# rvp-group/mad-icp

Hardware: NVIDIA H100
Metric: scans/sec (130k-pt scan vs 16-keyframe model) (higher is better)
Workload: dtype f64

## Files before the change

### include/madicp_b200.h

```cpp
#ifndef MADICP_B200_H
#define MADICP_B200_H

#include <stddef.h>
#include <stdint.h>

#ifdef __cplusplus
extern "C" {
#endif

#define MADICP_OK 0
#define MADICP_ERR_INVALID (-1)
#define MADICP_ERR_CUDA (-2)
#define MADICP_ERR_STATE (-3)
#define MADICP_ERR_NOMEM (-4)
#define MADICP_ERR_COMM (-5)

#define MADICP_MAX_ITERS 64

typedef struct madtree_rec {
  double mean[3];
  double dir[3];
  double bbox0;
  int32_t link;
  int32_t num_points;
// ... 56 lines not shown
int madicp_get_moving(madicp_ctx_t* ctx, double* means_out, int cap_leaves);
int madicp_put_keyframe_tree(madicp_ctx_t* ctx, int slot, const madtree_gpu_t* t, const double X[12]);

int madicp_ingest(madicp_ctx_t* ctx, const void* xyz, int64_t n, int is_f32, int deskew, const double T_prev[12],
                  const double T_now[12], double sensor_hz, int num_threads, double* points_out);

int madicp_search(madicp_ctx_t* ctx, const double X[12], int32_t* out_ordinals);

int madicp_linearize(madicp_ctx_t* ctx, const double X[12], double H[36], double b[6], uint8_t* matched);

int madicp_solve_update(madicp_ctx_t* ctx, const double H[36], const double b[6], double X_inout[12]);

int madicp_register(madicp_ctx_t* ctx, int iters, double X_inout[12], double H_last[36], double b_last[6],
                    uint8_t* matched_last, int* n_matched);
int madicp_register_async(madicp_ctx_t* ctx, int iters, const double X0[12]);
int madicp_register_fetch(madicp_ctx_t* ctx, double X[12], double H_last[36], double b_last[6], uint8_t* matched_last,
                          int* n_matched);
int madicp_register_fetch_weight(madicp_ctx_t* ctx, double X[12], double H_last[36], double b_last[6],
                                 uint8_t* matched_last, int* n_matched, double* weight);
int madicp_register_partial_async(madicp_ctx_t* ctx, int iters, const double X0[12]);
int madicp_register_trace(madicp_ctx_t* ctx, double* X_trace, int max_rounds);

int madicp_register_walked(madicp_ctx_t* ctx, int32_t* walked, int max_rounds);

int madicp_deskew(double* points_xyz, int64_t n, const double T_prev[12], const double T_now[12], double sensor_hz,
                  int num_threads);

int madicp_search_cloud(madicp_ctx_t* ctx, int slot, const double* queries_xyz, int64_t n, int32_t* ordinals,
                        double* points, double* normals, double* dists);

int64_t madicp_kernel_launches(const madicp_ctx_t* ctx);
int64_t madicp_model_nodes(const madicp_ctx_t* ctx);

#define MADICP_IPC_HANDLE_BYTES 64
int madicp_comm_export(madicp_ctx_t* ctx, void* handle_out );
int madicp_comm_connect(madicp_ctx_t* ctx, int rank, int world, const void* all_handles );
int madicp_comm_world(const madicp_ctx_t* ctx);

int madicp_calibrate(madicp_ctx_t* ctx, const double X0[12]);


#ifdef __cplusplus
}
#endif
#endif
```

### include/madicp_b200_debug.h

```cpp
#ifndef MADICP_B200_DEBUG_H
#define MADICP_B200_DEBUG_H

#include "madicp_b200.h"

#ifdef __cplusplus
extern "C" {
#endif

int madicp_debug_timing(madicp_ctx_t* ctx, int enable, int64_t* out, int max_rounds);
int madicp_debug_cta_cycles(madicp_ctx_t* ctx, int64_t* out, int cap);
int madicp_debug_cta_stamps(madicp_ctx_t* ctx, int plane, int64_t* out, int cap);
int madicp_set_gn_grid(madicp_ctx_t* ctx, int threads_per_cta, int ctas_per_sm);


int madicp_debug_set_memo(madicp_ctx_t* ctx, int enable);

int64_t madicp_debug_sort_check(int64_t n, uint32_t seed, int64_t distinct, int num_threads);

#ifdef __cplusplus
}
#endif
#endif
```

### mad_icp_b200/_capi.py

```python
import ctypes as C
import os

import numpy as np

_HERE = os.path.dirname(os.path.abspath(__file__))
LIB_PATH = os.path.join(_HERE, "lib", "libmadicp_b200.so")
_lib = None

dp = C.POINTER(C.c_double)
ip = C.POINTER(C.c_int32)
bp = C.POINTER(C.c_uint8)
vp = C.c_void_p

SYMBOLS = {
    "madicp_last_error": (C.c_char_p, []),
    "madicp_abi_version": (C.c_int, []),
    "madtree_build": (C.c_int, [dp, C.c_int64, C.c_double, C.c_double, C.c_int, C.POINTER(vp)]),
    "madtree_free": (None, [vp]),
    "madtree_num_nodes": (C.c_int, [vp]),
    "madtree_num_leaves": (C.c_int, [vp]),
    "madtree_apply_transform": (C.c_int, [vp, dp]),
    "madtree_leaves": (C.c_int, [vp, dp, dp, dp, ip]),
    "madtree_records": (vp, [vp]),
    "madtree_num_levels": (C.c_int, [vp]),
# ... 22 lines not shown
    "madtree_gpu_num_leaves": (C.c_int, [vp]),
    "madtree_gpu_num_levels": (C.c_int, [vp]),
    "madtree_gpu_download": (C.c_int, [vp, vp, ip]),
    "madtree_gpu_export": (C.c_int, [vp, dp, dp, dp, ip]),
    "madicp_set_moving_tree": (C.c_int, [vp, vp]),
    "madicp_get_moving": (C.c_int, [vp, dp, C.c_int]),
    "madicp_ingest": (C.c_int, [vp, vp, C.c_int64, C.c_int, C.c_int, dp, dp, C.c_double, C.c_int, dp]),
    "madicp_register_fetch_weight": (C.c_int, [vp, dp, dp, dp, bp, C.POINTER(C.c_int), dp]),
    "madicp_register_partial_async": (C.c_int, [vp, C.c_int, dp]),
    "madicp_calibrate": (C.c_int, [vp, dp]),
    "madicp_drop_keyframe": (C.c_int, [vp, C.c_int]),
    "madicp_num_keyframes": (C.c_int, [vp]),
    "madicp_active_slots": (C.c_int, [vp, ip, C.c_int]),
    "madicp_keyframe_leaves": (C.c_int, [vp, C.c_int]),
    "madicp_set_moving": (C.c_int, [vp, vp, C.c_int]),
    "madicp_search": (C.c_int, [vp, dp, ip]),
    "madicp_linearize": (C.c_int, [vp, dp, dp, dp, bp]),
    "madicp_solve_update": (C.c_int, [vp, dp, dp, dp]),
    "madicp_register": (C.c_int, [vp, C.c_int, dp, dp, dp, bp, C.POINTER(C.c_int)]),
    "madicp_register_async": (C.c_int, [vp, C.c_int, dp]),
    "madicp_register_fetch": (C.c_int, [vp, dp, dp, dp, bp, C.POINTER(C.c_int)]),
    "madicp_register_trace": (C.c_int, [vp, dp, C.c_int]),
    "madicp_register_walked": (C.c_int, [vp, ip, C.c_int]),
    "madicp_search_cloud": (C.c_int, [vp, C.c_int, dp, C.c_int64, ip, dp, dp, dp]),
    "madicp_deskew": (C.c_int, [dp, C.c_int64, dp, dp, C.c_double, C.c_int]),
    "madicp_debug_sort_check": (C.c_int64, [C.c_int64, C.c_uint32, C.c_int64, C.c_int]),
    "madicp_kernel_launches": (C.c_int64, [vp]),
    "madicp_model_nodes": (C.c_int64, [vp]),
    "madicp_comm_export": (C.c_int, [vp, vp]),
    "madicp_comm_connect": (C.c_int, [vp, C.c_int, C.c_int, vp]),
    "madicp_comm_world": (C.c_int, [vp]),
    "madicp_debug_timing": (C.c_int, [vp, C.c_int, C.POINTER(C.c_int64), C.c_int]),
    "madicp_debug_cta_cycles": (C.c_int, [vp, C.POINTER(C.c_int64), C.c_int]),
    "madicp_set_gn_grid": (C.c_int, [vp, C.c_int, C.c_int]),
    "madicp_debug_set_memo": (C.c_int, [vp, C.c_int]),
    "madicp_debug_cta_stamps": (C.c_int, [vp, C.c_int, C.POINTER(C.c_int64), C.c_int]),
}

REC_DTYPE = np.dtype([("mean", "<f8", 3), ("dir", "<f8", 3), ("bbox0", "<f8"), ("link", "<i4"), ("num_points", "<i4")])
assert REC_DTYPE.itemsize == 64


class MadIcpError(RuntimeError):
    pass


# ... 43 lines not shown
```

### mad_icp_b200/csrc/capi.cu

```cuda
#include <cooperative_groups.h>
#include <cuda_runtime.h>

#include <algorithm>
#include <cmath>
#include <cstdio>
#include <cstdlib>
#include <cstring>
#include <new>
#include <stdexcept>
#include <string>
#include <vector>

#include "../../include/madicp_b200_debug.h"
#include "ctx.hpp"
#include "device_kernels.cuh"

namespace madicp {

static thread_local std::string g_error;
void set_error(const std::string& msg) { g_error = msg; }

}

using namespace madicp;
// ... 218 lines not shown
  c->max_keyframes = max_keyframes;
  c->sm_count = prop.multiProcessorCount;
  c->slots.resize(max_keyframes);
  {
    int lo_pri = 0, hi_pri = 0;
    CK(cudaDeviceGetStreamPriorityRange(&lo_pri, &hi_pri));
    CK(cudaStreamCreateWithPriority(&c->own_stream, cudaStreamNonBlocking, hi_pri));
  }
  c->stream = c->own_stream;
  CK(cudaMalloc(&c->d_state, sizeof(GnState)));
  CK(cudaMemset(c->d_state, 0, sizeof(GnState)));
  CK(cudaMalloc(&c->d_X, sizeof(double) * 64));
  CK(cudaMalloc(&c->d_comm, sizeof(CommBlock)));
  CK(cudaMemset(c->d_comm, 0, sizeof(CommBlock)));
  CK(cudaEventCreateWithFlags(&c->tree_free_ev, cudaEventDisableTiming));
  CK(cudaMalloc(&c->d_pool_lvl, size_t(max_keyframes) * (kMaxLevels + 1) * sizeof(int)));
  CK(cudaMalloc(&c->d_xform, size_t(madicp_ctx::kXformRing) * 12 * sizeof(double)));
  CK(cudaMallocHost(&c->h_xform, size_t(madicp_ctx::kXformRing) * 12 * sizeof(double)));
  CK(cudaMallocHost(&c->h_lvl, size_t(madicp_ctx::kXformRing) * (kMaxLevels + 1) * sizeof(int)));
  for (int i = 0; i < madicp_ctx::kXformRing; ++i) CK(cudaEventCreateWithFlags(&c->xform_done[i], cudaEventDisableTiming));
  CK(cudaMallocHost(&c->h_pinned, sizeof(double) * 64));
  CK(cudaMallocHost(&c->h_state, sizeof(GnState)));
  CK(cudaMallocHost(&c->h_matched, kMatchedCap));
  if (const char* e = getenv("MADICP_NO_MEMO")) c->use_memo = (atoi(e) == 0);
  int threads = 1024, ctas = 1;
  if (const char* e = getenv("MADICP_GN_SHAPE"))
    if (sscanf(e, "%d,%d", &threads, &ctas) == 2) c->gn_auto = false;
  int rc = configure_gn(c, threads, ctas);
  if (rc) return rc;
  c->cap_partial = size_t(c->sm_count) * 8 * kAcc;
  CK(cudaMalloc(&c->d_partial, c->cap_partial * sizeof(double)));
  CK(cudaMalloc(&c->d_tiles, c->cap_partial * sizeof(LLCell)));
  CK(cudaMemset(c->d_tiles, 0, c->cap_partial * sizeof(LLCell)));
  c->peer_comm[0] = c->d_comm;
  *out = c;
  return MADICP_OK;
  MADICP_CATCH("madicp_create")
}

void madicp_destroy(madicp_ctx_t* c) {
  if (!c) return;
  cudaSetDevice(c->device);
  cudaStreamSynchronize(c->stream);
  for (int r = 0; r < c->world; ++r)
    if (c->world > 1 && r != c->rank && c->peer_comm[r]) cudaIpcCloseMemHandle(c->peer_comm[r]);
  madicp_gpu_build_release(c);
  for (madtree_gpu* t : c->tree_cache) delete t;
  for (void* slab : c->tree_slabs) cudaFree(slab);
  cudaFree(c->d_pool_recs);
  cudaFree(c->d_pool_child0);
  cudaFree(c->d_pool_rec_of);
  cudaFree(c->d_pool_lvl);
  cudaFree(c->d_quad);
  cudaFree(c->d_pool_ww);
  cudaFree(c->d_xform);
  cudaFree(c->d_dbg_cta);
  cudaFree(c->d_moving);
  cudaFree(c->d_mov4);
  cudaFree(c->d_step_matched);
  cudaFree(c->d_hit);
  cudaFree(c->d_ord);
  cudaFree(c->d_cloud_q);
  cudaFree(c->d_cloud_o);
  cudaFree(c->d_partial);
  cudaFree(c->d_tiles);
  cudaFree(c->d_memo_leaf);
  cudaFree(c->d_memo_margin);
  cudaFree(c->d_state);
  cudaFree(c->d_X);
  cudaFree(c->d_comm);
  cudaFree(c->d_dbg);
  cudaFreeHost(c->h_xform);
  cudaFreeHost(c->h_lvl);
  cudaFreeHost(c->h_pinned);
  cudaFreeHost(c->h_state);
  for (int i = 0; i < madicp_ctx::kXformRing; ++i)
    if (c->xform_done[i]) cudaEventDestroy(c->xform_done[i]);
  cudaFreeHost(c->h_matched);
  if (c->tree_free_ev) cudaEventDestroy(c->tree_free_ev);
  cudaStreamDestroy(c->own_stream);
  delete c;
}

int madicp_set_params(madicp_ctx_t* c, double min_ball, double rho_ker, double b_ratio) {
  if (!c || !(min_ball > 0) || rho_ker < 0) {
    set_error("madicp_set_params: bad arguments");
    return MADICP_ERR_INVALID;
  }
  const bool reweigh = (min_ball != c->P.min_ball);
  c->P.min_ball = min_ball;
// ... 503 lines not shown
  A.clear_from = clear_from;
  A.matched = c->d_comm->matched[mb];
  size_t map_bytes = 0;
  {
    const size_t per_cta = size_t(madicp_num_keyframes(c)) * (size_t(c->L) / size_t(c->gn_grid) + 8) * 4 + 128;
    auto bucket = [](size_t bytes) {
      const size_t kb[] = {8, 16, 32, 64, 100, 132, 164, 196, 228};
      for (size_t b : kb)
        if (bytes + 1024 <= b * 1024) return b;
      return size_t(1 << 20);
    };
    const size_t ctas = size_t(c->gn_grid / c->sm_count);
    if (per_cta <= kGnMapMaxBytes && c->L < (1 << 26) && bucket((c->gn_smem + per_cta) * ctas) == bucket(c->gn_smem * ctas))
      map_bytes = per_cta;
  }
  A.map_in_smem = map_bytes ? 1 : 0;
  {
    const size_t stride = ((size_t(c->max_keyframes) * (c->cap_moving / size_t(c->gn_grid) + 8)) + 31) & ~size_t(31);
    const size_t need = stride * size_t(c->gn_grid);
    if (need > c->cap_memo) {
      CK(cudaStreamSynchronize(c->stream));
      cudaFree(c->d_memo_leaf);
      cudaFree(c->d_memo_margin);
      c->d_memo_leaf = nullptr;
      c->d_memo_margin = nullptr;
      c->cap_memo = 0;
      const size_t cap = need + need / 4;
      CK(cudaMalloc(&c->d_memo_leaf, cap * sizeof(int)));
      CK(cudaMalloc(&c->d_memo_margin, cap * sizeof(float)));
      c->cap_memo = cap;
    }
    A.memo_leaf = c->d_memo_leaf;
    A.memo_margin = c->d_memo_margin;
    A.item_stride = int(stride);
    A.use_memo = c->use_memo ? 1 : 0;
    A.walk_buf = mb;
  }
  A.st = c->d_state;
  A.dbg = c->d_dbg;
  A.dbg_cta = c->d_dbg ? c->d_dbg_cta : nullptr;
  c->epoch += uint32_t(iters);
  A.pose_epoch = c->pose_epoch;
  c->pose_epoch += uint32_t(iters);
  memcpy(A.X0, X0, 12 * sizeof(double));
  A.tiles = c->d_tiles;
  A.zero_next = c->d_comm->matched[mb ^ 1];
  A.zero_bytes = int((std::min(kMatchedCap, c->cap_moving) + 15) & ~size_t(15));
  void* args[] = {&A};
  CK(cudaLaunchCooperativeKernel(c->gn_kernel, dim3(c->gn_grid), dim3(c->gn_threads), args, c->gn_smem + map_bytes, c->stream));
  c->launches++;
  c->last_iters = iters;
  c->call_seq++;
  return MADICP_OK;
}

int madicp_register_async(madicp_ctx_t* c, int iters, const double X0[12]) {
  return register_enqueue(c, iters, X0, iters - 1);
}
// ... 56 lines not shown
  return madicp_register_fetch(c, X, H, b, matched, n_matched);
}

int madicp_register_trace(madicp_ctx_t* c, double* X_trace, int max_rounds) {
  if (!c || !X_trace || c->last_iters < 1) return MADICP_ERR_INVALID;
  CK(cudaSetDevice(c->device));
  int rows = c->last_iters + 1;
  if (rows > max_rounds) rows = max_rounds;
  CK(cudaMemcpyAsync(c->h_state->X_trace, c->d_state->X_trace, size_t(rows) * 12 * sizeof(double),
                     cudaMemcpyDeviceToHost, c->stream));
  CK(cudaStreamSynchronize(c->stream));
  memcpy(X_trace, c->h_state->X_trace, size_t(rows) * 12 * sizeof(double));
  return rows;
}

int madicp_register_walked(madicp_ctx_t* c, int32_t* walked, int max_rounds) {
  if (!c || !walked || c->last_iters < 1) return MADICP_ERR_INVALID;
  CK(cudaSetDevice(c->device));
  int rows = std::min(c->last_iters, max_rounds);
  CK(cudaMemcpyAsync(c->h_state->walked[0], c->d_state->walked[(c->call_seq - 1u) & 1u], size_t(rows) * sizeof(int),
                     cudaMemcpyDeviceToHost, c->stream));
  CK(cudaStreamSynchronize(c->stream));
  memcpy(walked, c->h_state->walked[0], size_t(rows) * sizeof(int));
  return rows;
}

int madicp_search_cloud(madicp_ctx_t* c, int slot, const double* q, int64_t n, int32_t* ordinals, double* points,
                        double* normals, double* dists) {
  if (!c || !q || n < 1 || slot < 0 || slot >= c->max_keyframes || c->slots[slot].n_nodes == 0) {
    set_error("madicp_search_cloud: bad arguments or empty slot");
    return MADICP_ERR_INVALID;
  }
  CK(cudaSetDevice(c->device));
  if (size_t(n) > c->cap_cloud) {
    CK(cudaStreamSynchronize(c->stream));
    cudaFree(c->d_cloud_q);
    cudaFree(c->d_cloud_o);
    c->d_cloud_q = nullptr;
    c->d_cloud_o = nullptr;
    c->cap_cloud = 0;
    const size_t cap = size_t(n) + size_t(n) / 4 + 1024;
    CK(cudaMalloc(&c->d_cloud_q, cap * 10 * sizeof(double)));
    CK(cudaMalloc(&c->d_cloud_o, cap * sizeof(int)));
    c->cap_cloud = cap;
  }
  double* d_q = c->d_cloud_q;
// ... 124 lines not shown
  }
  return rows;
}

int madicp_debug_cta_cycles(madicp_ctx_t* c, int64_t* out, int cap) {
  if (!c || !out || !c->d_dbg_cta) return MADICP_ERR_INVALID;
  CK(cudaSetDevice(c->device));
  CK(cudaStreamSynchronize(c->stream));
  const int n = std::min(cap, c->last_iters * c->gn_grid);
  CK(cudaMemcpy(out, c->d_dbg_cta, size_t(n) * sizeof(long long), cudaMemcpyDeviceToHost));
  return c->gn_grid;
}

int madicp_debug_cta_stamps(madicp_ctx_t* c, int plane, int64_t* out, int cap) {
  if (!c || !out || !c->d_dbg_cta || plane < 0 || plane > 4) return MADICP_ERR_INVALID;
  CK(cudaSetDevice(c->device));
  CK(cudaStreamSynchronize(c->stream));
  const int n = std::min(cap, c->last_iters * c->gn_grid);
  CK(cudaMemcpy(out, c->d_dbg_cta + size_t(plane) * MADICP_MAX_ITERS * c->gn_grid, size_t(n) * sizeof(long long),
                cudaMemcpyDeviceToHost));
  return c->gn_grid;
}

int madicp_debug_set_memo(madicp_ctx_t* c, int enable) {
  if (!c) return MADICP_ERR_INVALID;
  c->use_memo = enable != 0;
  return MADICP_OK;
}

int madicp_set_gn_grid(madicp_ctx_t* c, int threads_per_cta, int ctas_per_sm) {
  if (!c || ctas_per_sm < 1) return MADICP_ERR_INVALID;
  CK(cudaSetDevice(c->device));
  if (threads_per_cta == 0) {
    c->gn_auto = true;
    return 0;
  }
  int rc = configure_gn(c, threads_per_cta, ctas_per_sm);
  if (rc) return rc;
  c->gn_auto = false;
  return c->gn_grid / c->sm_count;
}

}
```

### mad_icp_b200/csrc/ctx.hpp

```cpp
#pragma once
#include <cuda_runtime.h>

#include <atomic>
#include <mutex>
#include <new>
#include <stdexcept>
#include <string>
#include <vector>

#include "kernels.cuh"

namespace madicp {
void set_error(const std::string& msg);

constexpr int kMaxLevels = 4096;
struct Slot {
  int n_nodes = 0, n_leaves = 0, n_levels = 0;
};
constexpr size_t kMatchedCap = size_t(1) << 20;

struct CommBlock {
  Mailbox box;
  unsigned char matched[2][kMatchedCap];
};
// ... 40 lines not shown
  cudaEvent_t tree_free_ev = nullptr;
  std::mutex tree_mu;
  void* build_state = nullptr;
  long long* d_dbg_cta = nullptr;
  madicp::IcpParams P{0.2, 0.31622776601683794, 0.02};
  double* d_moving = nullptr;
  madicp::Moving4* d_mov4 = nullptr;
  bool mov4_stale = true;
  unsigned char* d_step_matched = nullptr;
  int L = 0;
  size_t cap_moving = 0;
  uint32_t call_seq = 0;
  int* d_hit = nullptr;
  int* d_ord = nullptr;
  size_t cap_items = 0;
  double* d_cloud_q = nullptr;
  int* d_cloud_o = nullptr;
  size_t cap_cloud = 0;
  double* d_partial = nullptr;
  madicp::LLCell* d_tiles = nullptr;
  size_t cap_partial = 0;
  int* d_memo_leaf = nullptr;
  float* d_memo_margin = nullptr;
  size_t cap_memo = 0;
  bool use_memo = true;
  madicp::GnState* d_state = nullptr;
  double* d_X = nullptr;
  madicp::CommBlock* d_comm = nullptr;
  double* h_pinned = nullptr;
  madicp::GnState* h_state = nullptr;
  unsigned char* h_matched = nullptr;
  int gn_grid = 0;
  bool gn_auto = true;
  int gn_threads = 1024;
  const void* gn_kernel = nullptr;
  size_t gn_smem = 0;
  static constexpr int kNumAutoShapes = 6;
  static constexpr int kAutoShapes[kNumAutoShapes] = {768, 1024, 896, 704, 640, 512};
  double pass_cost[kNumAutoShapes] = {5570.0, 8260.0, 7480.0, 5650.0, 5325.0, 4650.0};
  bool calibrated = false;
  int last_iters = 0;
  long long* d_dbg = nullptr;
  std::atomic<int64_t> launches{0};
  int rank = 0, world = 1;
  madicp::CommBlock* peer_comm[madicp::kMaxPeers] = {};
  uint32_t epoch = 0;
  uint32_t pose_epoch = 1;
};
// ... 25 lines not shown
```

### mad_icp_b200/csrc/device_kernels.cuh

```cuda
#pragma once
#include "kernels.cuh"

namespace madicp {


__device__ __forceinline__ int depth_of(const int* __restrict__ lvl, int n_levels, int i) {
  int lo = 0, hi = n_levels;
  while (hi - lo > 1) {
    const int mid = (lo + hi) >> 1;
    if (__ldg(lvl + mid) <= i) lo = mid; else hi = mid;
  }
  return lo;
}

__global__ void __launch_bounds__(kStepBlock)
k_slot_ingest(const madtree_rec_t* src, madtree_rec_t* dst, int n, const double* __restrict__ Xp,
              const int* __restrict__ lvl, int n_levels, int* __restrict__ flag) {
  const int i = blockIdx.x * kStepBlock + threadIdx.x;
  if (i >= n) return;
  Rec r = load_rec_plain(src + i);
  const int npts = src[i].num_points;
  int f = 0;
  if (r.link >= 0 && (depth_of(lvl, n_levels, i) & 1) == 0)
    f = (src[r.link].link >= 0 || src[r.link + 1].link >= 0) ? 1 : 0;
// ... 279 lines not shown
  }
  __syncthreads();
}

struct GnArgs {
  ModelView model;
  IcpParams P;
  PeerView peers;
  const Moving4* moving;
  int L;
  int iters;
  int clear_from;
  unsigned char* matched;
  unsigned char* peer_matched[kMaxPeers];
  LLCell* tiles;
  double X0[12];
  unsigned char* zero_next;
  int zero_bytes;
  GnState* st;
  int map_in_smem;
  uint32_t pose_epoch;
  int* memo_leaf;
  float* memo_margin;
  int item_stride;
  int walk_buf;
  int use_memo;
  long long* dbg;
  long long* dbg_cta;
};
__device__ __forceinline__ long long global_ns() {
  long long t;
  asm volatile("mov.u64 %0, %%globaltimer;" : "=l"(t));
  return t;
}

template <int THREADS, int CTAS>
__global__ void __launch_bounds__(THREADS, CTAS)
k_gn_loop(const __grid_constant__ GnArgs A) {
  constexpr int WARPS = THREADS / 32;
  extern __shared__ __align__(16) double s_dyn[];
  double* s_stage_all = s_dyn;
  double(*s_red)[64] = reinterpret_cast<double(*)[64]>(s_dyn);
  double(*s_peer)[kAcc] = reinterpret_cast<double(*)[kAcc]>(s_dyn + WARPS * 64);
  static_assert(WARPS * 64 + kMaxPeers * kAcc <= WARPS * kStageTile, "scratch must fit in the staging tiles");
  __shared__ double s_tot[kAcc];
  __shared__ double s_b[6];
  __shared__ double s_X[12], s_Xp[12];
  __shared__ int s_qn;
  __shared__ int s_count[WARPS];
  GnState* st = A.st;
  const unsigned L = unsigned(A.L);
  const unsigned total = unsigned(A.model.K) * L;
  const bool multi = A.peers.world > 1;
  const unsigned lane = threadIdx.x & 31;
  const unsigned warp = threadIdx.x >> 5;
  double* stage = s_stage_all + warp * kStageTile;
  constexpr unsigned kPieces = 4;
  unsigned p_lo[kPieces], p_n[kPieces];
  unsigned n_b = 0;
#pragma unroll
  const unsigned G = gridDim.x;
  const unsigned light = (G >= 8u) ? 3u : 0u;
  const uint64_t W8 = 8ull * G - light;
  for (unsigned p = 0; p < kPieces; ++p) {
    const unsigned s = (p & 1u) ? (G - 1u - blockIdx.x) : blockIdx.x;
    auto cum8 = [&](unsigned pos) -> uint64_t {
      if (p & 1u) return (pos >= G) ? W8 : 8ull * pos;
      return pos ? 8ull * pos - light : 0ull;
    };
    const uint64_t p0 = (uint64_t(L) * p) / kPieces, p1 = (uint64_t(L) * (p + 1)) / kPieces;
    const unsigned lo = unsigned(p0 + ((p1 - p0) * cum8(s)) / W8);
// ... 12 lines not shown
      ++k;
    }
    const unsigned j = q;
    q = p_lo[kPieces - 1] + (j - (n_b - p_n[kPieces - 1]));
    unsigned acc = 0;
#pragma unroll
    for (unsigned p = 0; p + 1 < kPieces; ++p) {
      if (j >= acc && j < acc + p_n[p]) q = p_lo[p] + (j - acc);
      acc += p_n[p];
    }
  };
  unsigned* s_map = A.map_in_smem ? reinterpret_cast<unsigned*>(s_dyn + WARPS * kStageTile) : nullptr;
  if (s_map) {
    for (unsigned t0 = warp * 32; t0 < t_total; t0 += THREADS) {
      unsigned k, q;
      item_of(t0, k, q);
      s_map[t0 + lane] = (k << 26) | q;
    }
    __syncwarp();
  }

  for (int i = (blockIdx.x * THREADS + threadIdx.x) * 16; i < A.zero_bytes; i += gridDim.x * THREADS * 16)
    *reinterpret_cast<uint4*>(A.zero_next + i) = make_uint4(0, 0, 0, 0);
  if (blockIdx.x == 0 && threadIdx.x < MADICP_MAX_ITERS) st->walked[A.walk_buf ^ 1][threadIdx.x] = 0;
  int* const memo_leaf = A.memo_leaf + size_t(blockIdx.x) * A.item_stride;
  float* const memo_margin = A.memo_margin + size_t(blockIdx.x) * A.item_stride;
  auto item_at = [&](unsigned t0, unsigned& k, unsigned& q) {
    if (s_map) {
      const unsigned pk = s_map[t0 + lane];
      k = pk >> 26;
      q = pk & 0x3ffffffu;
    } else {
      item_of(t0, k, q);
    }
  };

  for (int it = 0; it < A.iters; ++it) {
    if (threadIdx.x < 12) {
      double x;
      if (it == 0) {
        x = A.X0[threadIdx.x];
      } else {
        const uint32_t ep = A.pose_epoch + uint32_t(it);
        uint32_t lo, hi, f0, f1;
        do {
          ll_load(&st->X_ll[threadIdx.x], lo, f0, hi, f1);
        } while (f0 != ep || f1 != ep);
        x = __hiloint2double(int(hi), int(lo));
      }
      s_Xp[threadIdx.x] = s_X[threadIdx.x];
      s_X[threadIdx.x] = x;
      if (it == 0 && blockIdx.x == 0) st->X_trace[threadIdx.x] = x;
    }
    if (threadIdx.x == 32) s_qn = 0;
    __syncthreads();
    const bool last_round = (it == A.iters - 1);
    double c0 = 0.0, c1 = 0.0;
    long long t_begin = 0;
    if (A.dbg && threadIdx.x == 0) t_begin = clock64();
    const size_t dbg_plane = size_t(MADICP_MAX_ITERS) * gridDim.x, dbg_at = size_t(it) * gridDim.x + blockIdx.x;
    if (A.dbg_cta && threadIdx.x == 0) A.dbg_cta[dbg_plane + dbg_at] = global_ns();

    int n_walked = 0;
    for (unsigned t0 = warp * 32; t0 < t_total; t0 += THREADS) {
      unsigned k, q;
      item_at(t0, k, q);
      double v[kStage];
#pragma unroll
      for (int i = 0; i < kStage; ++i) v[i] = 0.0;
      const unsigned t = t0 + lane;
      if (t < t_total) {
        const Moving4 m = load_moving(A.moving + q);
        double mx, my, mz;
        iso_apply(s_X, m.px, m.py, m.pz, mx, my, mz);
        int leaf = -1;
        Rec f;
        double ww = 0.0;
        if (it > 0 && A.use_memo) {
          const float have = memo_margin[t];
          const int last = memo_leaf[t];
          f = load_rec(A.model.recs + last);
          ww = __ldg(A.model.ww + last);
          double bx, by, bz;
          iso_apply(s_Xp, m.px, m.py, m.pz, bx, by, bz);
          const double dx = mx - bx, dy = my - by, dz = mz - bz;
          const double moved = 1.0001 * sqrt(dx * dx + dy * dy + dz * dz) + 1e-9 + 1e-12 * (fabs(mx) + fabs(my) + fabs(mz));
          const double left = double(have) - moved;
          if (left > 0.0) {
            memo_margin[t] = __double2float_rd(left);
            leaf = last;
          }
        }
        if (leaf < 0) {
          double ww_walk;
          float margin = __int_as_float(0x7f800000);
          leaf = A.use_memo ? descend_t<true>(A.model, int(k), mx, my, mz, ww_walk, margin)
                            : descend_t<false>(A.model, int(k), mx, my, mz, ww_walk, margin);
          if (A.use_memo) {
            memo_leaf[t] = leaf;
            memo_margin[t] = margin;
          }
          ++n_walked;
          ww = __ldg(A.model.ww + leaf);
          f = load_rec(A.model.recs + leaf);
        }
        if (linearize_one(s_X, A.P.rho_ker_sqrt, m, mx, my, mz, f, ww, v) && it >= A.clear_from) {
          if (multi) {
            for (int r = 0; r < A.peers.world; ++r) A.peer_matched[r][q] = 1;
          } else {
            A.matched[q] = 1;
          }
        }
      }
      warp_accumulate(stage, v, c0, c1);
    }
    n_walked = __reduce_add_sync(0xffffffffu, n_walked);
    if (lane == 0 && n_walked) atomicAdd(&s_qn, n_walked);
    if (A.dbg && threadIdx.x == 0 && blockIdx.x == 0) A.dbg[it * 8 + 0] = clock64() - t_begin;
    if (A.dbg_cta) {
      __syncthreads();
      if (threadIdx.x == 0) {
        A.dbg_cta[dbg_at] = clock64() - t_begin;
        A.dbg_cta[2 * dbg_plane + dbg_at] = global_ns();
      }
      if (threadIdx.x == 0 && blockIdx.x == 0) A.dbg[it * 8 + 5] = s_qn;
    }
    __syncthreads();
    if (threadIdx.x == 0 && s_qn) atomicAdd(&st->walked[A.walk_buf][it], s_qn);
    const uint32_t ep_round = A.pose_epoch + uint32_t(it);
    block_reduce_publish<WARPS>(c0, c1, s_red, A.tiles + size_t(blockIdx.x) * kAcc, ep_round,
                                 it >= A.clear_from, multi);
    if (A.dbg_cta && threadIdx.x == 0) A.dbg_cta[3 * dbg_plane + dbg_at] = global_ns();
    if (blockIdx.x == 0) {
      long long t0 = 0, t1 = 0, t2 = 0;
      if (A.dbg && threadIdx.x == 0) t0 = clock64();
      fold_tiles<THREADS>(A.tiles, gridDim.x, ep_round, s_red, s_tot,
                          (A.dbg_cta && gridDim.x >= 16) ? A.dbg_cta + 4 * dbg_plane + size_t(it) * gridDim.x : nullptr);
      if (A.dbg && threadIdx.x == 0) {
        t1 = clock64();
        A.dbg[it * 8 + 1] = t1 - t_begin;
        A.dbg[it * 8 + 2] = t1 - t0;
        A.dbg[it * 8 + 6] = global_ns();
      }
      if (multi) {
        if (last_round) __threadfence_system();
        peer_allreduce<THREADS>(A.peers, A.peers.epoch_base + uint32_t(it) + 1u, s_tot, s_peer, &st->error);
        if (last_round) __threadfence_system();
      }
      if (last_round) {
        __threadfence();
        int c = 0;
// ... 54 lines not shown
```

### mad_icp_b200/csrc/kernels.cuh

```cuda
#pragma once
#include <cuda_runtime.h>
#include <stdint.h>

#include "../../include/madicp_b200.h"
#include "arith.h"
#include "solve6.h"

namespace madicp {

constexpr int kMaxSlots = 64;
constexpr int kStepBlock = 256;
constexpr int kAcc = 48;
constexpr int kStage = 13;
constexpr int kStageItems = 16;
constexpr int kStagePitch = 20;
constexpr int kStageTile = kStage * kStagePitch;
constexpr int kMaxPeers = 16;
constexpr int kMailboxSlots = 2;

struct __align__(16) FastRec {
  float dx, dy, dz, c;
};
static_assert(sizeof(FastRec) == 16, "FastRec must be one 128-bit load");

// ... 29 lines not shown
  uint32_t lo, flag_lo, hi, flag_hi;
};

__device__ __forceinline__ void ll_store(LLCell* p, double v, uint32_t epoch) {
  asm volatile("st.volatile.global.v4.u32 [%0], {%1,%2,%3,%4};" ::"l"(p), "r"(uint32_t(__double2loint(v))), "r"(epoch),
               "r"(uint32_t(__double2hiint(v))), "r"(epoch) : "memory");
}
__device__ __forceinline__ void ll_load(const LLCell* p, uint32_t& lo, uint32_t& f0, uint32_t& hi, uint32_t& f1) {
  asm volatile("ld.volatile.global.v4.u32 {%0,%1,%2,%3}, [%4];" : "=r"(lo), "=r"(f0), "=r"(hi), "=r"(f1) : "l"(p) : "memory");
}

struct GnState {
  int ticket;
  int clear_from;
  int n_matched;
  int error;
  double X_in[12];
  double X_out[12];
  double H[36];
  double b[6];
  double weight;
  double X_trace[(MADICP_MAX_ITERS + 1) * 12];
  int walked[2][MADICP_MAX_ITERS];
  LLCell X_ll[12];
};

struct Mailbox {
  LLCell cell[kMailboxSlots][kMaxPeers][kAcc];
};

struct PeerView {
  Mailbox* box[kMaxPeers];
  int rank, world;
  uint32_t epoch_base;
};

struct Rec {
  double mx, my, mz, dx, dy, dz, bbox0;
  int link;
};

__device__ __forceinline__ void ld_nc_f64x2(const void* p, double& a, double& b) {
  asm volatile("ld.global.nc.v2.f64 {%0,%1}, [%2];" : "=d"(a), "=d"(b) : "l"(p));
}
__device__ __forceinline__ void ld_nc_f32x4(const void* p, float& a, float& b, float& c, float& d) {
  asm volatile("ld.global.nc.v4.f32 {%0,%1,%2,%3}, [%4];" : "=f"(a), "=f"(b), "=f"(c), "=f"(d) : "l"(p));
// ... 61 lines not shown
  q.eq = __fmul_ru(kBoundC, __fadd_ru(__fadd_ru(fabsf(q.x), fabsf(q.y)), fabsf(q.z)));
  return q;
}
struct SideF {
  bool decided, right;
  float margin;
};
__device__ __forceinline__ SideF side_filtered2(const QueryF& q, const FastRec& p) {
  const float s = fmaf(q.z, p.dz, fmaf(q.y, p.dy, q.x * p.dx)) - p.c;
  const float E = __fmaf_ru(kBoundC, fabsf(p.c), q.eq);
  SideF r;
  r.decided = fabsf(s) > E;
  r.right = s > 0.0f;
  r.margin = __fsub_rd(fabsf(s), E);
  return r;
}
__device__ __forceinline__ bool is_leaf(const FastRec& p) { return __float_as_uint(p.dy) == kLeafMarker; }
__device__ __forceinline__ int leaf_index(const FastRec& p) { return __float_as_int(p.dx); }
__device__ __forceinline__ double leaf_weight(const FastRec& p) {
  return __hiloint2double(__float_as_int(p.c), __float_as_int(p.dz));
}

template <bool MEMO>
__device__ __forceinline__ int descend_t(const ModelView& M, int k, double qx, double qy, double qz, double& ww, float& margin) {
  const QueryF q = make_query(qx, qy, qz);
  const unsigned qroot = unsigned(M.qroot[k]);
  const QuadRec* qbase = M.quad;
  unsigned g = qroot;
  while (true) {
    FastRec p0, p1, p2;
    int bfs0, child0, pad1, pad2;
    const char* rp = reinterpret_cast<const char*>(qbase + g);
    ld_nc_f32x4(rp, p0.dx, p0.dy, p0.dz, p0.c);
    ld_nc_f32x4(rp + 16, p1.dx, p1.dy, p1.dz, p1.c);
    ld_nc_f32x4(rp + 32, p2.dx, p2.dy, p2.dz, p2.c);
    ld_nc_s32x4(rp + 48, bfs0, child0, pad1, pad2);
    if (is_leaf(p0)) {
      ww = leaf_weight(p0);
      return leaf_index(p0);
    }
    const SideF f0 = side_filtered2(q, p0);
    bool s0 = f0.right;
    if (MEMO) {
      float mg = f0.margin;
      if (!f0.decided) {
        const float r = side_exact_m(M.recs + bfs0, qx, qy, qz);
        s0 = exact_right(r);
        mg = fabsf(r);
      }
      margin = fminf(margin, mg);
    } else if (!f0.decided) {
      s0 = side_exact(M.recs + bfs0, qx, qy, qz);
// ... 1 lines not shown
    const FastRec c = s0 ? p2 : p1;
    if (is_leaf(c)) {
      ww = leaf_weight(c);
      return leaf_index(c);
    }
    const SideF f1 = side_filtered2(q, c);
    bool s1 = f1.right;
    if (MEMO) {
      float mg = f1.margin;
      if (!f1.decided) {
        const float r = side_exact_m(M.recs + (M.broot[k] + load_rec_link(M.recs + bfs0) + (s0 ? 1 : 0)), qx, qy, qz);
        s1 = exact_right(r);
        mg = fabsf(r);
      }
      margin = fminf(margin, mg);
    } else if (!f1.decided) {
      s1 = side_exact(M.recs + (M.broot[k] + load_rec_link(M.recs + bfs0) + (s0 ? 1 : 0)), qx, qy, qz);
    }
    g = qroot + unsigned(child0) + (s0 ? 2u : 0u) + (s1 ? 1u : 0u);
  }
}

__device__ __forceinline__ int descend(const ModelView& M, int k, double qx, double qy, double qz, double& ww) {
  float unused = 0.0f;
  return descend_t<false>(M, k, qx, qy, qz, ww, unused);
}

__device__ __forceinline__ bool linearize_one(const double* __restrict__ X, double rho, const Moving4& m, double mlx,
                                              double mly, double mlz, const Rec& f, double ww, double* v) {
  const double ex = mlx - f.mx, ey = mly - f.my, ez = mlz - f.mz;
  const double d2 = dot3(ex, ey, ez, ex, ey, ez);
  const double b2 = m.ball * m.ball;
  if (d2 > b2 * (1.0 + 1e-14)) return false;
  if (!(d2 < b2 * (1.0 - 1e-14)) && sqrt(d2) > m.ball) return false;
  const double e = fma(ez, f.dz, fma(ey, f.dy, ex * f.dx));
  double J[6];
  J[0] = fma(f.dz, X[8], fma(f.dy, X[4], f.dx * X[0]));
  J[1] = fma(f.dz, X[9], fma(f.dy, X[5], f.dx * X[1]));
  J[2] = fma(f.dz, X[10], fma(f.dy, X[6], f.dx * X[2]));
  J[3] = fma(J[2], m.py, -(J[1] * m.pz));
  J[4] = fma(J[0], m.pz, -(J[2] * m.px));
  J[5] = fma(J[1], m.px, -(J[0] * m.py));
  double scale = ww;
  const double chi = fabs(e);
  if (chi > rho) scale = (rho / chi) * ww;
#pragma unroll
  for (int i = 0; i < 6; ++i) {
    v[i] = scale * J[i];
// ... 179 lines not shown
```

### mad_icp_b200/engine.py

```python
import ctypes as C

import numpy as np

from . import _capi as capi
from ._capi import MadIcpError, as_b, as_d, as_i, check, pose12


class FlatTree:

    def __init__(self, points, b_max=0.2, b_min=0.1, num_threads=1):
        pts = np.ascontiguousarray(points, dtype=np.float64)
        if pts.ndim != 2 or pts.shape[1] != 3:
            raise ValueError("points must be N x 3")
        h = C.c_void_p()
        check(capi.lib().madtree_build(as_d(pts), pts.shape[0], b_max, b_min, num_threads, C.byref(h)), "madtree_build")
        self._h = h
        self.b_max, self.b_min = b_max, b_min

    def __del__(self):
        h = getattr(self, "_h", None)
        if h:
            self._h = None
            try:
                capi.lib().madtree_free(h)
# ... 250 lines not shown
    def register_async(self, X0, iters=15, partial=False):
        X = pose12(X0)
        fn = capi.lib().madicp_register_partial_async if partial else capi.lib().madicp_register_async
        check(fn(self._h, iters, as_d(X)), "madicp_register_async")

    def register_fetch(self, want_matched=False):
        X, H, b = np.empty((3, 4)), np.empty((6, 6)), np.empty(6)
        m = np.empty(self.L, np.uint8) if want_matched else None
        n, w = C.c_int(0), C.c_double(0)
        check(capi.lib().madicp_register_fetch_weight(self._h, as_d(X), as_d(H), as_d(b), as_b(m), C.byref(n), C.byref(w)),
              "madicp_register_fetch")
        return dict(X=X, H=H, b=b, matched=m, n_matched=n.value, weight=w.value)

    def register_trace(self):
        buf = np.empty((65, 3, 4))
        rows = check(capi.lib().madicp_register_trace(self._h, as_d(buf), 65), "madicp_register_trace")
        return buf[:rows].copy()

    def register_walked(self):
        buf = np.zeros(64, np.int32)
        rows = check(capi.lib().madicp_register_walked(self._h, as_i(buf), 64), "madicp_register_walked")
        return buf[:rows].copy()

    def search_cloud(self, slot, queries, want=("ordinals", "points", "normals", "dists")):
        q = np.ascontiguousarray(queries, dtype=np.float64).reshape(-1, 3)
        n = q.shape[0]
        o = np.empty(n, np.int32) if "ordinals" in want else None
        p = np.empty((n, 3)) if "points" in want else None
        nr = np.empty((n, 3)) if "normals" in want else None
        d = np.empty(n) if "dists" in want else None
        check(capi.lib().madicp_search_cloud(self._h, slot, as_d(q), n, as_i(o), as_d(p), as_d(nr), as_d(d)),
              "madicp_search_cloud")
        return dict(ordinals=o, points=p, normals=nr, dists=d)

    def debug_timing(self, enable=True, fetch=True):
        buf = np.zeros((64, 8), np.int64)
        rows = check(capi.lib().madicp_debug_timing(self._h, int(enable), buf.ctypes.data_as(C.POINTER(C.c_int64))
                                                    if fetch else None, 64))
        return buf[:rows]

    def debug_cta_cycles(self, rounds):
        buf = np.zeros(rounds * 2048, np.int64)
        grid = check(capi.lib().madicp_debug_cta_cycles(self._h, buf.ctypes.data_as(C.POINTER(C.c_int64)), buf.size))
        return buf[:rounds * grid].reshape(rounds, grid)

    def debug_cta_stamps(self, plane, rounds):
        buf = np.zeros(rounds * 2048, np.int64)
        grid = check(capi.lib().madicp_debug_cta_stamps(self._h, plane, buf.ctypes.data_as(C.POINTER(C.c_int64)), buf.size))
        return buf[:rounds * grid].reshape(rounds, grid)

    def set_memo(self, enable=True):
        check(capi.lib().madicp_debug_set_memo(self._h, int(enable)))

    def set_gn_grid(self, threads_per_cta=1024, ctas_per_sm=1):
        return check(capi.lib().madicp_set_gn_grid(self._h, threads_per_cta, ctas_per_sm))

    def comm_export(self):
        buf = (C.c_char * 64)()
        check(capi.lib().madicp_comm_export(self._h, buf), "madicp_comm_export")
        return bytes(buf)

    def comm_connect(self, rank, world, handles):
        blob = b"".join(handles)
        assert len(blob) == 64 * world
        check(capi.lib().madicp_comm_connect(self._h, rank, world, blob), "madicp_comm_connect")

    @property
    def world(self):
        return capi.lib().madicp_comm_world(self._h)


__all__ = ["FlatTree", "DeviceTree", "Registrar", "MadIcpError"]
```

Measured before the change: 4685.

## Resume tree descent from memoized checkpoint when leaf memo margin is exhausted

Adds a second memo level: during each descent the kernel records the deepest tree node whose safety margin still exceeds a motion-based threshold. On later Gauss-Newton iterations, when the cached leaf is no longer valid, the walk restarts from that checkpoint rather than from the root, which cuts node visits per query. The cost is two extra per-item arrays (checkpoint index and margin slack), extra loads and stores, and a per-node comparison and record counter inside the descent loop. A walk-record counter API is also added for diagnostics.

```diff
diff --git a/include/madicp_b200.h b/include/madicp_b200.h
--- a/include/madicp_b200.h
+++ b/include/madicp_b200.h
@@ -102,6 +102,7 @@
 int madicp_register_trace(madicp_ctx_t* ctx, double* X_trace, int max_rounds);
 
 int madicp_register_walked(madicp_ctx_t* ctx, int32_t* walked, int max_rounds);
+int madicp_register_walk_records(madicp_ctx_t* ctx, int64_t* records, int max_rounds);
 
 int madicp_deskew(double* points_xyz, int64_t n, const double T_prev[12], const double T_now[12], double sensor_hz,
                   int num_threads);
diff --git a/include/madicp_b200_debug.h b/include/madicp_b200_debug.h
--- a/include/madicp_b200_debug.h
+++ b/include/madicp_b200_debug.h
@@ -13,7 +13,7 @@
 int madicp_set_gn_grid(madicp_ctx_t* ctx, int threads_per_cta, int ctas_per_sm);
 
 
-int madicp_debug_set_memo(madicp_ctx_t* ctx, int enable);
+int madicp_debug_set_memo(madicp_ctx_t* ctx, int mode);
 
 int64_t madicp_debug_sort_check(int64_t n, uint32_t seed, int64_t distinct, int num_threads);
 
diff --git a/mad_icp_b200/_capi.py b/mad_icp_b200/_capi.py
--- a/mad_icp_b200/_capi.py
+++ b/mad_icp_b200/_capi.py
@@ -68,6 +68,7 @@
     "madicp_register_fetch": (C.c_int, [vp, dp, dp, dp, bp, C.POINTER(C.c_int)]),
     "madicp_register_trace": (C.c_int, [vp, dp, C.c_int]),
     "madicp_register_walked": (C.c_int, [vp, ip, C.c_int]),
+    "madicp_register_walk_records": (C.c_int, [vp, C.POINTER(C.c_int64), C.c_int]),
     "madicp_search_cloud": (C.c_int, [vp, C.c_int, dp, C.c_int64, ip, dp, dp, dp]),
     "madicp_deskew": (C.c_int, [dp, C.c_int64, dp, dp, C.c_double, C.c_int]),
     "madicp_debug_sort_check": (C.c_int64, [C.c_int64, C.c_uint32, C.c_int64, C.c_int]),
diff --git a/mad_icp_b200/csrc/capi.cu b/mad_icp_b200/csrc/capi.cu
--- a/mad_icp_b200/csrc/capi.cu
+++ b/mad_icp_b200/csrc/capi.cu
@@ -264,7 +264,7 @@
   CK(cudaMallocHost(&c->h_pinned, sizeof(double) * 64));
   CK(cudaMallocHost(&c->h_state, sizeof(GnState)));
   CK(cudaMallocHost(&c->h_matched, kMatchedCap));
-  if (const char* e = getenv("MADICP_NO_MEMO")) c->use_memo = (atoi(e) == 0);
+  if (const char* e = getenv("MADICP_NO_MEMO")) c->memo_mode = (atoi(e) == 0) ? 2 : 0;
   int threads = 1024, ctas = 1;
   if (const char* e = getenv("MADICP_GN_SHAPE"))
     if (sscanf(e, "%d,%d", &threads, &ctas) == 2) c->gn_auto = false;
@@ -308,6 +308,8 @@
   cudaFree(c->d_tiles);
   cudaFree(c->d_memo_leaf);
   cudaFree(c->d_memo_margin);
+  cudaFree(c->d_memo_ckpt);
+  cudaFree(c->d_memo_ckpt_up);
   cudaFree(c->d_state);
   cudaFree(c->d_X);
   cudaFree(c->d_comm);
@@ -857,18 +859,26 @@
       CK(cudaStreamSynchronize(c->stream));
       cudaFree(c->d_memo_leaf);
       cudaFree(c->d_memo_margin);
+      cudaFree(c->d_memo_ckpt);
+      cudaFree(c->d_memo_ckpt_up);
       c->d_memo_leaf = nullptr;
       c->d_memo_margin = nullptr;
+      c->d_memo_ckpt = nullptr;
+      c->d_memo_ckpt_up = nullptr;
       c->cap_memo = 0;
       const size_t cap = need + need / 4;
       CK(cudaMalloc(&c->d_memo_leaf, cap * sizeof(int)));
       CK(cudaMalloc(&c->d_memo_margin, cap * sizeof(float)));
+      CK(cudaMalloc(&c->d_memo_ckpt, cap * sizeof(unsigned)));
+      CK(cudaMalloc(&c->d_memo_ckpt_up, cap * sizeof(float)));
       c->cap_memo = cap;
     }
     A.memo_leaf = c->d_memo_leaf;
     A.memo_margin = c->d_memo_margin;
+    A.memo_ckpt = c->d_memo_ckpt;
+    A.memo_ckpt_up = c->d_memo_ckpt_up;
     A.item_stride = int(stride);
-    A.use_memo = c->use_memo ? 1 : 0;
+    A.memo_mode = c->memo_mode;
     A.walk_buf = mb;
   }
   A.st = c->d_state;
@@ -971,6 +981,17 @@
                      cudaMemcpyDeviceToHost, c->stream));
   CK(cudaStreamSynchronize(c->stream));
   memcpy(walked, c->h_state->walked[0], size_t(rows) * sizeof(int));
+  return rows;
+}
+
+int madicp_register_walk_records(madicp_ctx_t* c, int64_t* records, int max_rounds) {
+  if (!c || !records || c->last_iters < 1) return MADICP_ERR_INVALID;
+  CK(cudaSetDevice(c->device));
+  int rows = std::min(c->last_iters, max_rounds);
+  CK(cudaMemcpyAsync(c->h_state->walk_recs[0], c->d_state->walk_recs[(c->call_seq - 1u) & 1u],
+                     size_t(rows) * sizeof(unsigned long long), cudaMemcpyDeviceToHost, c->stream));
+  CK(cudaStreamSynchronize(c->stream));
+  for (int i = 0; i < rows; ++i) records[i] = int64_t(c->h_state->walk_recs[0][i]);
   return rows;
 }
 
@@ -1141,9 +1162,12 @@
   return c->gn_grid;
 }
 
-int madicp_debug_set_memo(madicp_ctx_t* c, int enable) {
-  if (!c) return MADICP_ERR_INVALID;
-  c->use_memo = enable != 0;
+int madicp_debug_set_memo(madicp_ctx_t* c, int mode) {
+  if (!c || mode < 0 || mode > 2) {
+    set_error("madicp_debug_set_memo: mode must be 0 (off), 1 (leaf memo) or 2 (leaf memo + resume)");
+    return MADICP_ERR_INVALID;
+  }
+  c->memo_mode = mode;
   return MADICP_OK;
 }
 
diff --git a/mad_icp_b200/csrc/ctx.hpp b/mad_icp_b200/csrc/ctx.hpp
--- a/mad_icp_b200/csrc/ctx.hpp
+++ b/mad_icp_b200/csrc/ctx.hpp
@@ -86,8 +86,10 @@
   size_t cap_partial = 0;
   int* d_memo_leaf = nullptr;
   float* d_memo_margin = nullptr;
+  unsigned* d_memo_ckpt = nullptr;
+  float* d_memo_ckpt_up = nullptr;
   size_t cap_memo = 0;
-  bool use_memo = true;
+  int memo_mode = 2;
   madicp::GnState* d_state = nullptr;
   double* d_X = nullptr;
   madicp::CommBlock* d_comm = nullptr;
diff --git a/mad_icp_b200/csrc/device_kernels.cuh b/mad_icp_b200/csrc/device_kernels.cuh
--- a/mad_icp_b200/csrc/device_kernels.cuh
+++ b/mad_icp_b200/csrc/device_kernels.cuh
@@ -325,12 +325,21 @@
   uint32_t pose_epoch;
   int* memo_leaf;
   float* memo_margin;
+  unsigned* memo_ckpt;
+  float* memo_ckpt_up;
   int item_stride;
   int walk_buf;
-  int use_memo;
+  int memo_mode;
   long long* dbg;
   long long* dbg_cta;
 };
+#ifndef MADICP_CKPT_TAU_SCALE
+#define MADICP_CKPT_TAU_SCALE 1.0
+#endif
+__device__ __forceinline__ float ckpt_tau(int it, double moved, double ball) {
+  return __double2float_ru(MADICP_CKPT_TAU_SCALE * (it == 0 ? ball : moved));
+}
+
 __device__ __forceinline__ long long global_ns() {
   long long t;
   asm volatile("mov.u64 %0, %%globaltimer;" : "=l"(t));
@@ -349,7 +358,7 @@
   __shared__ double s_tot[kAcc];
   __shared__ double s_b[6];
   __shared__ double s_X[12], s_Xp[12];
-  __shared__ int s_qn;
+  __shared__ int s_qn, s_rn;
   __shared__ int s_count[WARPS];
   GnState* st = A.st;
   const unsigned L = unsigned(A.L);
@@ -408,9 +417,14 @@
 
   for (int i = (blockIdx.x * THREADS + threadIdx.x) * 16; i < A.zero_bytes; i += gridDim.x * THREADS * 16)
     *reinterpret_cast<uint4*>(A.zero_next + i) = make_uint4(0, 0, 0, 0);
-  if (blockIdx.x == 0 && threadIdx.x < MADICP_MAX_ITERS) st->walked[A.walk_buf ^ 1][threadIdx.x] = 0;
+  if (blockIdx.x == 0 && threadIdx.x < MADICP_MAX_ITERS) {
+    st->walked[A.walk_buf ^ 1][threadIdx.x] = 0;
+    st->walk_recs[A.walk_buf ^ 1][threadIdx.x] = 0;
+  }
   int* const memo_leaf = A.memo_leaf + size_t(blockIdx.x) * A.item_stride;
   float* const memo_margin = A.memo_margin + size_t(blockIdx.x) * A.item_stride;
+  unsigned* const memo_ckpt = A.memo_ckpt + size_t(blockIdx.x) * A.item_stride;
+  float* const memo_ckpt_up = A.memo_ckpt_up + size_t(blockIdx.x) * A.item_stride;
   auto item_at = [&](unsigned t0, unsigned& k, unsigned& q) {
     if (s_map) {
       const unsigned pk = s_map[t0 + lane];
@@ -439,6 +453,7 @@
       if (it == 0 && blockIdx.x == 0) st->X_trace[threadIdx.x] = x;
     }
     if (threadIdx.x == 32) s_qn = 0;
+    if (threadIdx.x == 33) s_rn = 0;
     __syncthreads();
     const bool last_round = (it == A.iters - 1);
     double c0 = 0.0, c1 = 0.0;
@@ -447,7 +462,7 @@
     const size_t dbg_plane = size_t(MADICP_MAX_ITERS) * gridDim.x, dbg_at = size_t(it) * gridDim.x + blockIdx.x;
     if (A.dbg_cta && threadIdx.x == 0) A.dbg_cta[dbg_plane + dbg_at] = global_ns();
 
-    int n_walked = 0;
+    int n_walked = 0, n_recs = 0;
     for (unsigned t0 = warp * 32; t0 < t_total; t0 += THREADS) {
       unsigned k, q;
       item_at(t0, k, q);
@@ -462,29 +477,50 @@
         int leaf = -1;
         Rec f;
         double ww = 0.0;
-        if (it > 0 && A.use_memo) {
+        unsigned start = 0;
+        float prefix = __int_as_float(0x7f800000);
+        double moved = 0.0;
+        if (it > 0 && A.memo_mode) {
           const float have = memo_margin[t];
           const int last = memo_leaf[t];
+          unsigned ck = 0;
+          float ck_up = 0.0f;
+          if (A.memo_mode == 2) {
+            ck = memo_ckpt[t];
+            ck_up = memo_ckpt_up[t];
+          }
           f = load_rec(A.model.recs + last);
           ww = __ldg(A.model.ww + last);
           double bx, by, bz;
           iso_apply(s_Xp, m.px, m.py, m.pz, bx, by, bz);
           const double dx = mx - bx, dy = my - by, dz = mz - bz;
-          const double moved = 1.0001 * sqrt(dx * dx + dy * dy + dz * dz) + 1e-9 + 1e-12 * (fabs(mx) + fabs(my) + fabs(mz));
+          moved = 1.0001 * sqrt(dx * dx + dy * dy + dz * dz) + 1e-9 + 1e-12 * (fabs(mx) + fabs(my) + fabs(mz));
           const double left = double(have) - moved;
           if (left > 0.0) {
             memo_margin[t] = __double2float_rd(left);
             leaf = last;
+          } else if (ck != 0) {
+            const double ck_left = __dsub_rd(__dadd_rd(double(have), double(ck_up)), moved);
+            if (ck_left > 0.0) {
+              start = ck;
+              prefix = __double2float_rd(ck_left);
+            }
           }
         }
         if (leaf < 0) {
           double ww_walk;
-          float margin = __int_as_float(0x7f800000);
-          leaf = A.use_memo ? descend_t<true>(A.model, int(k), mx, my, mz, ww_walk, margin)
-                            : descend_t<false>(A.model, int(k), mx, my, mz, ww_walk, margin);
-          if (A.use_memo) {
+          const float tau = ckpt_tau(it, moved, m.ball);
+          float margin = prefix, ck_margin = 0.0f;
+          unsigned ckpt = start;
+          leaf = A.memo_mode ? descend_t<true>(A.model, int(k), mx, my, mz, ww_walk, margin, ckpt, ck_margin, tau, n_recs)
+                             : descend_t<false>(A.model, int(k), mx, my, mz, ww_walk, margin, ckpt, ck_margin, tau, n_recs);
+          if (A.memo_mode) {
             memo_leaf[t] = leaf;
             memo_margin[t] = margin;
+          }
+          if (A.memo_mode == 2) {
+            memo_ckpt[t] = ckpt;
+            memo_ckpt_up[t] = __fsub_rd(ck_margin, margin);
           }
           ++n_walked;
           ww = __ldg(A.model.ww + leaf);
@@ -501,7 +537,11 @@
       warp_accumulate(stage, v, c0, c1);
     }
     n_walked = __reduce_add_sync(0xffffffffu, n_walked);
-    if (lane == 0 && n_walked) atomicAdd(&s_qn, n_walked);
+    n_recs = __reduce_add_sync(0xffffffffu, n_recs);
+    if (lane == 0 && n_walked) {
+      atomicAdd(&s_qn, n_walked);
+      atomicAdd(&s_rn, n_recs);
+    }
     if (A.dbg && threadIdx.x == 0 && blockIdx.x == 0) A.dbg[it * 8 + 0] = clock64() - t_begin;
     if (A.dbg_cta) {
       __syncthreads();
@@ -512,7 +552,10 @@
       if (threadIdx.x == 0 && blockIdx.x == 0) A.dbg[it * 8 + 5] = s_qn;
     }
     __syncthreads();
-    if (threadIdx.x == 0 && s_qn) atomicAdd(&st->walked[A.walk_buf][it], s_qn);
+    if (threadIdx.x == 0 && s_qn) {
+      atomicAdd(&st->walked[A.walk_buf][it], s_qn);
+      atomicAdd(&st->walk_recs[A.walk_buf][it], (unsigned long long) s_rn);
+    }
     const uint32_t ep_round = A.pose_epoch + uint32_t(it);
     block_reduce_publish<WARPS>(c0, c1, s_red, A.tiles + size_t(blockIdx.x) * kAcc, ep_round,
                                  it >= A.clear_from, multi);
diff --git a/mad_icp_b200/csrc/kernels.cuh b/mad_icp_b200/csrc/kernels.cuh
--- a/mad_icp_b200/csrc/kernels.cuh
+++ b/mad_icp_b200/csrc/kernels.cuh
@@ -75,6 +75,7 @@
   double weight;
   double X_trace[(MADICP_MAX_ITERS + 1) * 12];
   int walked[2][MADICP_MAX_ITERS];
+  unsigned long long walk_recs[2][MADICP_MAX_ITERS];
   LLCell X_ll[12];
 };
 
@@ -182,12 +183,19 @@
 }
 
 template <bool MEMO>
-__device__ __forceinline__ int descend_t(const ModelView& M, int k, double qx, double qy, double qz, double& ww, float& margin) {
+__device__ __forceinline__ int descend_t(const ModelView& M, int k, double qx, double qy, double qz, double& ww, float& margin,
+                                         unsigned& ckpt, float& ckpt_margin, float tau, int& n_rec) {
   const QueryF q = make_query(qx, qy, qz);
   const unsigned qroot = unsigned(M.qroot[k]);
   const QuadRec* qbase = M.quad;
-  unsigned g = qroot;
+  unsigned g = qroot + ckpt;
+  if (MEMO) ckpt_margin = margin;
   while (true) {
+    if (MEMO && margin >= tau) {
+      ckpt = g - qroot;
+      ckpt_margin = margin;
+    }
+    ++n_rec;
     FastRec p0, p1, p2;
     int bfs0, child0, pad1, pad2;
     const char* rp = reinterpret_cast<const char*>(qbase + g);
@@ -235,8 +243,10 @@
 }
 
 __device__ __forceinline__ int descend(const ModelView& M, int k, double qx, double qy, double qz, double& ww) {
-  float unused = 0.0f;
-  return descend_t<false>(M, k, qx, qy, qz, ww, unused);
+  float unused = 0.0f, unused_ck = 0.0f;
+  unsigned root = 0;
+  int unused_n = 0;
+  return descend_t<false>(M, k, qx, qy, qz, ww, unused, root, unused_ck, 0.0f, unused_n);
 }
 
 __device__ __forceinline__ bool linearize_one(const double* __restrict__ X, double rho, const Moving4& m, double mlx,
diff --git a/mad_icp_b200/engine.py b/mad_icp_b200/engine.py
--- a/mad_icp_b200/engine.py
+++ b/mad_icp_b200/engine.py
@@ -296,6 +296,12 @@
         rows = check(capi.lib().madicp_register_walked(self._h, as_i(buf), 64), "madicp_register_walked")
         return buf[:rows].copy()
 
+    def register_walk_records(self):
+        buf = np.zeros(64, np.int64)
+        rows = check(capi.lib().madicp_register_walk_records(self._h, buf.ctypes.data_as(C.POINTER(C.c_int64)), 64),
+                     "madicp_register_walk_records")
+        return buf[:rows].copy()
+
     def search_cloud(self, slot, queries, want=("ordinals", "points", "normals", "dists")):
         q = np.ascontiguousarray(queries, dtype=np.float64).reshape(-1, 3)
         n = q.shape[0]
@@ -323,8 +329,10 @@
         grid = check(capi.lib().madicp_debug_cta_stamps(self._h, plane, buf.ctypes.data_as(C.POINTER(C.c_int64)), buf.size))
         return buf[:rounds * grid].reshape(rounds, grid)
 
-    def set_memo(self, enable=True):
-        check(capi.lib().madicp_debug_set_memo(self._h, int(enable)))
+    def set_memo(self, mode=True):
+        if isinstance(mode, bool):
+            mode = 2 if mode else 0
+        check(capi.lib().madicp_debug_set_memo(self._h, int(mode)), "madicp_debug_set_memo")
 
     def set_gn_grid(self, threads_per_cta=1024, ctas_per_sm=1):
         return check(capi.lib().madicp_set_gn_grid(self._h, threads_per_cta, ctas_per_sm))
```

Result: faster. 4992 (median of 6 runs) (+6.6%).
